# codihuston/eioku

Hardware: AMD Instinct MI355X
Metric: frames/sec (scene+detect+embed) per node (higher is better)
Workload: dtype f16

## Files before the change

eioku_amd/csrc/knn.hip:

```cpp
#include "common.h"
#include "select.h"

#include <cstdlib>

#include <cfloat>

using namespace eioku;

namespace {

constexpr int kQT = 32;
constexpr int kRT = 32;
constexpr int kWaves = 4;

template <int K>
struct TopK {
  float v[K];
  int id[K];
  __device__ __forceinline__ void init() {
#pragma unroll
    for (int p = 0; p < K; ++p) {
      v[p] = FLT_MAX;
      id[p] = 0x7FFFFFFF;
    }
// ... 262 lines not shown
  const float ra = a - __uint_as_float(ua & 0xFFFF0000u), rb = b - __uint_as_float(ub & 0xFFFF0000u);
  lo = (__float_as_uint(ra) >> 16) | (__float_as_uint(rb) & 0xFFFF0000u);
}

template <int K, int D>
__global__ __launch_bounds__(256, 1) void k_flat_l2_bf(KnnArgs a) {
  if (a.gate && *a.gate == 0) return;
  constexpr int KC = D < 128 ? D : 128;
  constexpr int NCH = D / KC;
  constexpr int NS = KC / 16;
  constexpr int PPR = KC / 8;
  constexpr int UPR = 2 * PPR;
  constexpr int TILE_U = kRT * UPR;
  constexpr int SPT = kRT * (KC / 4) / 256;
  constexpr int LISTS = 2, NQ_WG = kQT * kWaves;
  constexpr size_t STAGE_B = (size_t)2 * NCH * TILE_U * 16 + (size_t)2 * kRT * 4;
  constexpr size_t MERGE_B = (size_t)NQ_WG * LISTS * K * 8;
  static_assert(KC % 16 == 0 && D % KC == 0 && (kRT * (KC / 4)) % 256 == 0, "tile shape");
  __shared__ __attribute__((aligned(16))) unsigned char smem[STAGE_B > MERGE_B ? STAGE_B : MERGE_B];
  u32x4k* lds = reinterpret_cast<u32x4k*>(smem);
  float* lnorm = reinterpret_cast<float*>(smem + (size_t)2 * NCH * TILE_U * 16);

  const int tid = threadIdx.x, lane = tid & 63, wave = tid >> 6;
  const int col = lane & 31, half = lane >> 5;
  const int qt = blockIdx.y * kWaves + wave;
  const int qi = qt * kQT + col;
  const bool qvalid = qi < a.nq;

  u32x4k Qh[D / 16], Ql[D / 16];
  {
    const float* qp = a.q + (size_t)(qvalid ? qi : 0) * D + 8 * half;
#pragma unroll
    for (int s = 0; s < D / 16; ++s) {
      const float4 v0 = *reinterpret_cast<const float4*>(qp + 16 * s);
      const float4 v1 = *reinterpret_cast<const float4*>(qp + 16 * s + 4);
      unsigned h[4], l[4];
      split_bf16x2(v0.x, v0.y, h[0], l[0]);
      split_bf16x2(v0.z, v0.w, h[1], l[1]);
      split_bf16x2(v1.x, v1.y, h[2], l[2]);
      split_bf16x2(v1.z, v1.w, h[3], l[3]);
      Qh[s] = qvalid ? u32x4k{h[0], h[1], h[2], h[3]} : u32x4k{0, 0, 0, 0};
      Ql[s] = qvalid ? u32x4k{l[0], l[1], l[2], l[3]} : u32x4k{0, 0, 0, 0};
    }
  }
  const float qn = qvalid ? a.qnorm[qi] : 0.f;
  TopK<K> top;
  top.init();

  const long long slab0 = (long long)blockIdx.x * a.slab_stride;
  const long long slab1 = min(a.n, slab0 + a.rows_per_block);
  float4 stage[2][NCH][SPT];
  float stage_n[2] = {0.f, 0.f};
  auto issue = [&](long long row0, int slot) {
#pragma unroll
    for (int ch = 0; ch < NCH; ++ch)
#pragma unroll
      for (int it = 0; it < SPT; ++it) {
        const int id = tid + 256 * it;
        long long r = row0 + id / (KC / 4);
        if (r >= slab1) r = slab1 - 1;
        stage[slot][ch][it] = *reinterpret_cast<const float4*>(a.db + (size_t)r * D + ch * KC + (id % (KC / 4)) * 4);
      }
    long long r = row0 + (tid < kRT ? tid : 0);
    if (r >= slab1) r = slab1 - 1;
    stage_n[slot] = a.dbnorm[r];
  };
  auto commit = [&](int buf, int slot) {
#pragma unroll
    for (int ch = 0; ch < NCH; ++ch)
#pragma unroll
      for (int it = 0; it < SPT; ++it) {
        const int id = tid + 256 * it;
        const int row = id / (KC / 4), fu = id % (KC / 4);
        const int p = (fu >> 1) ^ (row & (PPR - 1) & 15), sub = fu & 1;
        unsigned h0, l0, h1, l1;
        split_bf16x2(stage[slot][ch][it].x, stage[slot][ch][it].y, h0, l0);
        split_bf16x2(stage[slot][ch][it].z, stage[slot][ch][it].w, h1, l1);
        const u32x2k hi = u32x2k{h0, h1}, lo = u32x2k{l0, l1};
        unsigned char* base = reinterpret_cast<unsigned char*>(lds + (buf * NCH + ch) * TILE_U + row * UPR);
        *reinterpret_cast<u32x2k*>(base + p * 16 + sub * 8) = hi;
        *reinterpret_cast<u32x2k*>(base + (PPR + p) * 16 + sub * 8) = lo;
      }
    if (tid < kRT) lnorm[buf * kRT + tid] = stage_n[slot];
  };
  auto multiply = [&](long long row0, int buf) {
    f32x16 acc;
#pragma unroll
    for (int r = 0; r < 16; ++r) acc[r] = 0.f;
#pragma unroll
    for (int ch = 0; ch < NCH; ++ch) {
      const u32x4k* rowp = lds + (buf * NCH + ch) * TILE_U + col * UPR;
      u32x4k xh[NS], xl[NS];
#pragma unroll
      for (int s = 0; s < NS; ++s) {
        const int p = (2 * s + half) ^ (col & (PPR - 1) & 15);
        xh[s] = rowp[p];
        xl[s] = rowp[PPR + p];
      }
#pragma unroll
      for (int s = 0; s < NS; ++s) {
        const bf16x8 h = __builtin_bit_cast(bf16x8, xh[s]), l = __builtin_bit_cast(bf16x8, xl[s]);
        const bf16x8 qh = __builtin_bit_cast(bf16x8, Qh[ch * NS + s]), ql = __builtin_bit_cast(bf16x8, Ql[ch * NS + s]);
        acc = __builtin_amdgcn_mfma_f32_32x32x16_bf16(h, qh, acc, 0, 0, 0);
        acc = __builtin_amdgcn_mfma_f32_32x32x16_bf16(l, qh, acc, 0, 0, 0);
        acc = __builtin_amdgcn_mfma_f32_32x32x16_bf16(h, ql, acc, 0, 0, 0);
      }
      __builtin_amdgcn_sched_group_barrier(0x100, 4, 0);
#pragma unroll
      for (int s = 0; s < NS; ++s) {
        __builtin_amdgcn_sched_group_barrier(0x008, 3, 0);
        __builtin_amdgcn_sched_group_barrier(0x100, 2, 0);
      }
    }
#pragma unroll
    for (int r = 0; r < 16; ++r) {
      const int lr = (r & 3) + 8 * (r >> 2) + 4 * half;
      const long long row = row0 + lr;
      if (row < slab1) {
        float dist = (qn + lnorm[buf * kRT + lr]) - 2.0f * acc[r];
        dist = dist < 0.f ? 0.f : dist;
        const int id = (int)(row - slab0);
        if (top.beats_tail(dist, id)) top.insert(dist, id);
      }
    }
  };

  long long row0 = slab0;
  if (row0 < slab1) {
    issue(row0, 0);
    issue(row0 + kRT, 1);
    commit(0, 0);
  }
  __syncthreads();
  while (row0 < slab1) {
#pragma unroll
    for (int par = 0; par < 2; ++par) {
      if (row0 >= slab1) break;
      issue(row0 + 2 * kRT, par);
      multiply(row0, par);
      commit(par ^ 1, par ^ 1);
      __syncthreads();
      row0 += kRT;
    }
  }

  __syncthreads();
  float (*s_mv)[LISTS][K] = reinterpret_cast<float (*)[LISTS][K]>(smem);
  int (*s_mi)[LISTS][K] = reinterpret_cast<int (*)[LISTS][K]>(smem + (size_t)NQ_WG * LISTS * K * 4);
  {
    const int ql = wave * kQT + col;
#pragma unroll
    for (int p = 0; p < K; ++p) {
      s_mv[ql][half][p] = top.v[p];
      s_mi[ql][half][p] = top.id[p];
    }
  }
  __syncthreads();
  if (tid < NQ_WG) {
    int head[LISTS] = {0, 0};
    const int qtile = blockIdx.y * kWaves + tid / kQT;
    const size_t out = (((size_t)qtile * gridDim.x + blockIdx.x) * kQT + (tid % kQT)) * K;
    for (int p = 0; p < K; ++p) {
      float bv = FLT_MAX;
      int bi = 0x7FFFFFFF, bl = 0;
#pragma unroll
      for (int l = 0; l < LISTS; ++l) {
        if (head[l] < K) {
          const float v = s_mv[tid][l][head[l]];
          const int i = s_mi[tid][l][head[l]];
          if (v < bv || (v == bv && i < bi)) {
            bv = v;
            bi = i;
            bl = l;
          }
        }
      }
#pragma unroll
      for (int l = 0; l < LISTS; ++l)
        if (l == bl) head[l]++;
      a.pd[out + p] = bv;
      a.pi[out + p] = bi == 0x7FFFFFFF ? -1 : bi;
    }
  }
}

__global__ __launch_bounds__(256) void k_row_norms(const float* x, long long n, int d, float* out) {
  const int lane = threadIdx.x & 63;
  long long row = (blockIdx.x * 256ll + threadIdx.x) >> 6;
  const long long nw = ((long long)gridDim.x * 256) >> 6;
  for (; row < n; row += nw) {
    float s = 0.f;
    for (int c = lane * 4; c < d; c += 256) {
      const float4 v = *reinterpret_cast<const float4*>(x + (size_t)row * d + c);
      s += v.x * v.x;
      s += v.y * v.y;
      s += v.z * v.z;
      s += v.w * v.w;
    }
#pragma unroll
    for (int off = 32; off > 0; off >>= 1) s += __shfl_xor(s, off, 64);
    if (lane == 0) out[row] = s;
  }
}

template <int K>
__global__ __launch_bounds__(64) void k_topk_merge(const float* pd, const int* pi, const long long* pi64,
                                                   int L, int nq, int kin, int qstride_lists,
                                                   const long long* list_base, long long rows_per_list,
                                                   int k, float* D, long long* I, const int* gate = nullptr) {
  if (gate && *gate == 0) return;
  const int q = blockIdx.x, lane = threadIdx.x;
  SmallTop<K> top;
  top.init();
  for (int l = lane; l < L; l += 64) {
    size_t base;
    if (qstride_lists > 0) base = ((((size_t)(q / kQT) * L + l) * kQT) + (q % kQT)) * kin;
    else base = ((size_t)l * nq + q) * kin;
    for (int p = 0; p < kin; ++p) {
      const float v = pd[base + p];
      long long id;
      if (pi64) id = pi64[base + p];
      else {
        const int li = pi[base + p];
        id = li < 0 ? -1 : (long long)li + (list_base ? list_base[l] : (long long)l * rows_per_list);
      }
      if (id < 0) break;
      if (!top.better(v, id, top.v[K - 1], top.id[K - 1])) break;
      top.insert(v, id);
    }
  }
  for (int r = 0; r < k; ++r) {
    float bv = top.id[0] < 0 ? FLT_MAX : top.v[0];
    long long bi = top.id[0] < 0 ? none<long long>() : top.id[0];
    int bl = lane;
    wave_argmin(bv, bi, bl);
    const bool found = bi != none<long long>();
    if (lane == 0) {
      D[(size_t)q * k + r] = found ? bv : FLT_MAX;
      I[(size_t)q * k + r] = found ? bi : -1;
    }
    if (found && lane == bl) {
#pragma unroll
      for (int s = 0; s < K - 1; ++s) {
        top.v[s] = top.v[s + 1];
        top.id[s] = top.id[s + 1];
      }
      top.v[K - 1] = FLT_MAX;
      top.id[K - 1] = -1;
    }
  }
}

__global__ __launch_bounds__(64) void k_topk_merge_heads(const float* __restrict__ pd, const int* __restrict__ pi, int L, int kin,
                                                         long long rows_per_list, int k, float* __restrict__ D,
                                                         long long* __restrict__ I, const int* __restrict__ gate) {
  if (gate && *gate == 0) return;
  const int q = blockIdx.x, lane = threadIdx.x;
  const bool have = lane < L;
  const size_t base = ((((size_t)(q / kQT) * L + (have ? lane : 0)) * kQT) + (q % kQT)) * kin;
  const long long idb = (long long)lane * rows_per_list;
  int h = 0;
  float cv = FLT_MAX, nv = FLT_MAX;
  int ci = -1, ni = -1;
  if (have) {
    cv = pd[base];
    ci = pi[base];
    if (kin > 1) {
      nv = pd[base + 1];
      ni = pi[base + 1];
    }
  }
  for (int r = 0; r < k; ++r) {
    float bv = ci < 0 ? FLT_MAX : cv;
    long long bi = ci < 0 ? none<long long>() : (long long)ci + idb;
    int bl = lane;
    wave_argmin(bv, bi, bl);
    const bool found = bi != none<long long>();
    if (lane == 0) {
      D[(size_t)q * k + r] = found ? bv : FLT_MAX;
      I[(size_t)q * k + r] = found ? bi : -1;
    }
    if (found && lane == bl) {
      ++h;
      cv = nv;
      ci = ni;
      if (h + 1 < kin && ni >= 0) {
        nv = pd[base + h + 1];
        ni = pi[base + h + 1];
      } else {
        ni = -1;
      }
    }
  }
}

template <int D, int SPLIT>
__global__ __launch_bounds__(256) void k_split_planes(const float* __restrict__ x, long long n, long long first_tile,
                                                      const float* __restrict__ norms, u32x4k* __restrict__ hi,
                                                      float* __restrict__ hnorm, float* __restrict__ tmax) {
  constexpr int NS = D / 16, PU = NS * 64;
  const long long tile = first_tile + blockIdx.x / SPLIT;
  const int part = blockIdx.x % SPLIT;
  for (int o = part * (PU / SPLIT) + threadIdx.x; o < (part + 1) * (PU / SPLIT); o += 256) {
    const int s = o >> 6, h = (o >> 5) & 1, r = o & 31;
    const long long row = tile * 32 + r;
    float v[8];
    if (row < n) {
      const float4 a = *reinterpret_cast<const float4*>(x + (size_t)row * D + 16 * s + 8 * h);
      const float4 b = *reinterpret_cast<const float4*>(x + (size_t)row * D + 16 * s + 8 * h + 4);
      v[0] = a.x; v[1] = a.y; v[2] = a.z; v[3] = a.w; v[4] = b.x; v[5] = b.y; v[6] = b.z; v[7] = b.w;
    } else {
#pragma unroll
      for (int j = 0; j < 8; ++j) v[j] = 0.f;
    }
    unsigned hb[8];
#pragma unroll
    for (int j = 0; j < 8; ++j) hb[j] = bf16_rne_bits(v[j]);
    hi[(size_t)tile * PU + o] = u32x4k{hb[0] | (hb[1] << 16), hb[2] | (hb[3] << 16), hb[4] | (hb[5] << 16), hb[6] | (hb[7] << 16)};
  }
  if (hnorm && part == 0 && threadIdx.x < 64) {
    const int r = threadIdx.x & 31;
    const long long row = tile * 32 + r;
    const float nn = row < n ? norms[row] : 0.f;
    if (threadIdx.x < 32) hnorm[tile * 32 + r] = row < n ? 0.5f * nn : __builtin_inff();
    float m = nn < __builtin_inff() ? sqrtf(nn) : 0.f;
#pragma unroll
    for (int off = 16; off > 0; off >>= 1) m = fmaxf(m, __shfl_xor(m, off, 64));
    if (threadIdx.x == 0) tmax[tile] = m;
  }
}

struct ScanArgs {
  const u32x4k* xh;
  const float* hnorm;
  const float* tmax;
  const float* xmax;
  const u32x4k* qh;
  const float* qnorm;
  const float* tau;
  int tau_k;
  long long n, ntiles;
  long long tstride;
  int nq, nqt;
  unsigned* wl;
  int* wl_cnt;
  int wl_cap;
};

template <int D, int NW, int RT>
__global__ __launch_bounds__(NW * 64) void k_l2_scan(ScanArgs a) {
  constexpr int NS = D / 16, PU = NS * 64;
  constexpr int NDMA = (PU / 64 + NW - 1) / NW;
  extern __shared__ __attribute__((aligned(16))) unsigned char dyn_smem[];
  constexpr int NB = 4;
  u32x4k* qbuf = reinterpret_cast<u32x4k*>(dyn_smem);
  float* s_hc = reinterpret_cast<float*>(dyn_smem + (size_t)NB * PU * 16);
  float* s_sq = s_hc + a.nqt * 32;
  float* s_hx = s_sq + a.nqt * 32;
  int* s_cnt = reinterpret_cast<int*>(s_hx + NW * RT * 32);

  const int tid = threadIdx.x, lane = tid & 63;
  const int wave = __builtin_amdgcn_readfirstlane(tid >> 6);
  const int col = lane & 31, half = lane >> 5;

  for (int q = tid; q < a.nqt * 32; q += NW * 64) {
    float hc = __builtin_inff(), sq = 0.f;
    if (q < a.nq) {
      const float t = a.tau[(size_t)q * a.tau_k + (a.tau_k - 1)];
      const float qn = a.qnorm[q];
      const float nrm = sqrtf(qn) + a.xmax[0];
      hc = 0.5f * (qn - (t + 2e-5f * (1.0f + t) + 1e-6f * nrm * nrm));
      sq = 0.0078125f * 1.002f * sqrtf(qn);
    }
    s_hc[q] = hc;
    s_sq[q] = sq;
  }
  if (tid == 0) *s_cnt = 0;
  unsigned* const my_list = a.wl + (size_t)blockIdx.x * a.wl_cap * 2;

  const long long nwt = (a.ntiles + NW * RT - 1) / (NW * RT);
  auto stage_q = [&](int qt, int buf) {
#pragma unroll
    for (int j = 0; j < NDMA; ++j) {
      int u = (j * NW + wave) * 64;
      if (u >= PU) u = PU - 64;
      __builtin_amdgcn_global_load_lds((gbl_cvoid_t*)(a.qh + (size_t)qt * PU + u + lane),
                                       (lds_void_t*)(qbuf + (size_t)buf * PU + u), 16, 0, 0);
    }
  };

  u32x4k xh[RT][NS];
  float sxm[RT], hxmin[RT];
  long long wt = blockIdx.x;
  auto tile_of = [&](long long w, int i) {
    const long long t = (w * NW + wave) * RT + i;
    return (t < a.ntiles ? t : a.ntiles - 1) * a.tstride;
  };
  auto tile_min_hx = [&](long long t, int i) {
    float m = a.hnorm[t * 32 + col];
    if (half == 0) s_hx[(wave * RT + i) * 32 + col] = m;
#pragma unroll
    for (int off = 16; off > 0; off >>= 1) m = fminf(m, __shfl_xor(m, off, 64));
    return m;
  };
  const long long my_tiles = wt < nwt ? (nwt - 1 - wt) / gridDim.x + 1 : 0;
  const int total = (int)(my_tiles * a.nqt);
  if (wt < nwt) {
#pragma unroll
    for (int i = 0; i < RT; ++i) {
      const long long t = tile_of(wt, i);
#pragma unroll
      for (int s = 0; s < NS; ++s) xh[i][s] = a.xh[(size_t)t * PU + s * 64 + lane];
      sxm[i] = a.tmax[t];
      hxmin[i] = tile_min_hx(t, i);
    }
    __builtin_amdgcn_s_waitcnt(0x0f70);
    __builtin_amdgcn_sched_barrier(0);
    stage_q(0, 0);
    if (total > 1) stage_q(1 % a.nqt, 1);
  }
  int it = 0;
  int stage_qt = 2 % a.nqt;
  for (; wt < nwt; wt += gridDim.x) {
    bool own[RT];
    long long row0[RT], tn[RT];
    const long long nwt_next = wt + gridDim.x;
    const bool more_tiles = nwt_next < nwt;
#pragma unroll
    for (int i = 0; i < RT; ++i) {
      own[i] = (wt * NW + wave) * RT + i < a.ntiles;
      row0[i] = tile_of(wt, i) * 32;
      tn[i] = more_tiles ? tile_of(nwt_next, i) : 0;
    }
    for (int qt = 0; qt < a.nqt; ++qt, ++it) {
      const bool last_qt = qt == a.nqt - 1;
      const bool meet = (it & 1) == 0;
      if (meet || qt == 0) __builtin_amdgcn_s_waitcnt(0x0f70);
      if (meet) {
        __builtin_amdgcn_s_waitcnt(0xc07f);
        asm volatile("" ::: "memory");
        __builtin_amdgcn_s_barrier();
        asm volatile("" ::: "memory");
        __builtin_amdgcn_sched_barrier(0);
#pragma unroll
        for (int e = 2; e < 4; ++e) {
          if (it + e < total) stage_q(stage_qt, (it + e) & (NB - 1));
          stage_qt = stage_qt + 1 == a.nqt ? 0 : stage_qt + 1;
        }
      }
      __builtin_amdgcn_sched_barrier(0);
      const u32x4k* qb = qbuf + (size_t)(it & (NB - 1)) * PU;
      const float hcq = s_hc[qt * 32 + col];
      const float sqq = s_sq[qt * 32 + col];
      f32x16 acc[RT];
#pragma unroll
      for (int i = 0; i < RT; ++i)
#pragma unroll
        for (int r = 0; r < 16; ++r) acc[i][r] = 0.f;
      constexpr int PF = RT == 2 ? 2 : 4;
      u32x4k bh[PF];
#pragma unroll
      for (int s = 0; s < PF; ++s) bh[s] = qb[s * 64 + lane];
#pragma unroll
      for (int s = 0; s < NS; ++s) {
        const bf16x8 ch = __builtin_bit_cast(bf16x8, bh[s % PF]);
#pragma unroll
        for (int i = 0; i < RT; ++i)
          acc[i] = __builtin_amdgcn_mfma_f32_32x32x16_bf16(__builtin_bit_cast(bf16x8, xh[i][s]), ch, acc[i], 0, 0, 0);
        if (s + PF < NS) bh[s % PF] = qb[(s + PF) * 64 + lane];
        if (last_qt && more_tiles) {
#pragma unroll
          for (int i = 0; i < RT; ++i) {
            const unsigned char* base = reinterpret_cast<const unsigned char*>(a.xh) + ((size_t)tn[i] * PU + (s & ~3) * 64) * 16;
            asm volatile("global_load_dwordx4 %0, %1, %2 offset:%3" : "+v"(xh[i][s]) : "v"(lane * 16), "s"(base), "n"((s & 3) * 1024));
          }
        }
      }
      if (!last_qt) {
        __builtin_amdgcn_sched_group_barrier(0x100, PF, 0);
#pragma unroll
        for (int s = 0; s < NS; ++s) {
          __builtin_amdgcn_sched_group_barrier(0x008, RT, 0);
          __builtin_amdgcn_sched_group_barrier(0x100, 1, 0);
        }
      }
#pragma unroll
      for (int i = 0; i < RT; ++i) {
        const f32x16& c = acc[i];
        const float thr_q = hcq - sqq * sxm[i];
        auto ib = [&](int r) { return __float_as_int(c[r]); };
        const int i01 = max(max(ib(0), ib(1)), ib(2)), i23 = max(max(ib(3), ib(4)), ib(5));
        const int i45 = max(max(ib(6), ib(7)), ib(8)), i67 = max(max(ib(9), ib(10)), ib(11));
        const int i89 = max(max(ib(12), ib(13)), ib(14));
        const int imx = max(max(max(i01, i23), i45), max(max(i67, i89), ib(15)));
        const float T = hxmin[i] + thr_q;
        if ((!(T > 0.f) || imx >= __float_as_int(T)) && own[i]) {
          const int qi = qt * 32 + col;
          int h4 = 4 * half;
          asm volatile("" : "+v"(h4));
#pragma unroll
          for (int g = 0; g < 4; ++g) {
            const float4 hx = *reinterpret_cast<const float4*>(s_hx + (wave * RT + i) * 32 + 8 * g + h4);
#pragma unroll
            for (int j = 0; j < 4; ++j) {
              const float hxr = j == 0 ? hx.x : (j == 1 ? hx.y : (j == 2 ? hx.z : hx.w));
              if (c[4 * g + j] >= hxr + thr_q) {
                const int pos = atomicAdd(s_cnt, 1);
                if (pos < a.wl_cap) {
                  my_list[2 * (size_t)pos] = (unsigned)qi;
                  my_list[2 * (size_t)pos + 1] = (unsigned)((int)row0[i] + 8 * g + j + h4);
                }
              }
            }
          }
        }
      }
      if (last_qt && more_tiles) {
#pragma unroll
        for (int i = 0; i < RT; ++i) {
          sxm[i] = a.tmax[tn[i]];
          hxmin[i] = tile_min_hx(tn[i], i);
        }
      }
    }
  }
  __syncthreads();
  if (tid == 0) a.wl_cnt[blockIdx.x] = *s_cnt;
}

template <int D>
__global__ __launch_bounds__(256) void k_scan_select(const float* __restrict__ db, const float* __restrict__ q,
                                                     const int* __restrict__ cand_i, const int* __restrict__ cnt, int cap, int k,
                                                     float* __restrict__ Dout, long long* __restrict__ Iout,
                                                     int* __restrict__ overflow) {
  extern __shared__ __attribute__((aligned(16))) unsigned char dyn_smem[];
  float* sd = reinterpret_cast<float*>(dyn_smem);
  int* si = reinterpret_cast<int*>(sd + cap);
  __shared__ float s_bv[4];
  __shared__ int s_bi[4];
  const int qi = blockIdx.x, tid = threadIdx.x, lane = tid & 63;
  int c = cnt[qi];
  if (c > cap) {
    if (tid == 0) atomicOr(overflow, 1);
    c = cap;
  }
  for (int j = tid; j < c; j += 256) si[j] = cand_i[(size_t)qi * cap + j];
  __syncthreads();
  {
    constexpr int NV = D / 128, U = 4;
    const int l32 = lane & 31, hw = tid >> 5;
    float4 qv[NV];
#pragma unroll
    for (int t = 0; t < NV; ++t) qv[t] = *reinterpret_cast<const float4*>(q + (size_t)qi * D + 128 * t + 4 * l32);
    for (int j0 = hw; j0 < c; j0 += 8 * U) {
      float4 xv[U][NV];
#pragma unroll
      for (int u = 0; u < U; ++u) {
        const int j = j0 + 8 * u;
        const int r = si[j < c ? j : j0];
#pragma unroll
        for (int t = 0; t < NV; ++t) xv[u][t] = *reinterpret_cast<const float4*>(db + (size_t)r * D + 128 * t + 4 * l32);
      }
#pragma unroll
      for (int u = 0; u < U; ++u) {
        float sum = 0.f;
#pragma unroll
        for (int t = 0; t < NV; ++t) {
          float e;
          e = qv[t].x - xv[u][t].x; sum = fmaf(e, e, sum);
          e = qv[t].y - xv[u][t].y; sum = fmaf(e, e, sum);
          e = qv[t].z - xv[u][t].z; sum = fmaf(e, e, sum);
          e = qv[t].w - xv[u][t].w; sum = fmaf(e, e, sum);
        }
#pragma unroll
        for (int off = 16; off > 0; off >>= 1) sum += __shfl_xor(sum, off, 64);
        const int j = j0 + 8 * u;
        if (l32 == 0 && j < c) sd[j] = sum;
      }
    }
  }
  __syncthreads();
  float lv = -1.f;
  int li = -1;
  for (int r = 0; r < k; ++r) {
    float bv;
    int bi;
    next_after(lv, li, tid, c, 256, sd, si, bv, bi);
    block_argmin4(bv, bi, s_bv, s_bi);
    if (tid == 0) {
      Dout[(size_t)qi * k + r] = bi == none<int>() ? FLT_MAX : bv;
      Iout[(size_t)qi * k + r] = bi == none<int>() ? -1 : (long long)bi;
    }
    advance(lv, li, bv, bi);
  }
}

__global__ __launch_bounds__(1024) void k_sel_words(const unsigned* __restrict__ sel, const unsigned* __restrict__ live,
                                                    long long n, int nwords, unsigned* __restrict__ ew,
                                                    int* __restrict__ bcount) {
  __shared__ int s_cnt;
  if (threadIdx.x == 0) s_cnt = 0;
  __syncthreads();
  const int i = blockIdx.x * 1024 + threadIdx.x;
  unsigned w = 0;
  if (i < nwords) {
    w = sel ? sel[i] : 0xFFFFFFFFu;
    if (live) w &= live[i];
    const long long rem = n - (long long)i * 32;
    if (rem < 32) w &= (1u << (int)rem) - 1u;
    ew[i] = w;
  }
  const unsigned long long b = __ballot(w != 0);
  if ((threadIdx.x & 63) == 0 && b) atomicAdd(&s_cnt, __popcll(b));
  __syncthreads();
  if (threadIdx.x == 0) bcount[blockIdx.x] = s_cnt;
}

__global__ __launch_bounds__(1024) void k_sel_list(const unsigned* __restrict__ ew, const int* __restrict__ bcount, int nwords,
                                                   int* __restrict__ list, int* __restrict__ meta, long long ppm) {
  __shared__ int s_part[16], s_wc[16];
  const int tid = threadIdx.x, lane = tid & 63, wave = tid >> 6;
  int s = 0;
  for (int b = tid; b < (int)blockIdx.x; b += 1024) s += bcount[b];
#pragma unroll
  for (int off = 32; off > 0; off >>= 1) s += __shfl_xor(s, off, 64);
  const int i = blockIdx.x * 1024 + tid;
  const bool nz = i < nwords && ew[i] != 0;
  const unsigned long long b = __ballot(nz);
  if (lane == 0) {
    s_part[wave] = s;
    s_wc[wave] = __popcll(b);
  }
  __syncthreads();
  int base = 0, before = 0, mine = 0;
#pragma unroll
  for (int w = 0; w < 16; ++w) {
    base += s_part[w];
    before += w < wave ? s_wc[w] : 0;
    mine += s_wc[w];
  }
  if (nz) list[base + before + __popcll(b & ((1ull << lane) - 1ull))] = i;
  if (blockIdx.x == gridDim.x - 1 && tid == 0) {
    const int total = base + mine;
    const bool use_list = (long long)total * 1000000ll <= ppm * (long long)nwords;
    meta[0] = total;
    meta[1] = use_list ? 1 : 0;
    meta[2] = use_list ? 0 : 1;
  }
}

__global__ __launch_bounds__(256) void k_remove_ids(const long long* __restrict__ ids, long long n_ids, long long n,
                                                    long long planes_n, unsigned* __restrict__ live, float* __restrict__ norms,
                                                    float* __restrict__ hnorm, int* __restrict__ removed) {
  const long long i = blockIdx.x * 256ll + threadIdx.x;
  if (i >= n_ids) return;
  const long long id = ids[i];
  if (id < 0 || id >= n) return;
  const unsigned bit = 1u << (int)(id & 31);
  const unsigned old = atomicAnd(live + (id >> 5), ~bit);
  if (old & bit) {
    atomicAdd(removed, 1);
    norms[id] = __builtin_inff();
    if (hnorm && id < planes_n) hnorm[id] = __builtin_inff();
  }
}

}

struct eioku_index {
  int d = 0;
  long long n = 0;
  DevBuf<float> x_own;
  float* x = nullptr;
  DevBuf<float> norms;
  bool attached = false;
  long long cap() const { return attached ? n : (long long)(x_own.cap / d); }
  DevBuf<float> qbuf, qnorm, pd, dout;
  DevBuf<int> pi;
  DevBuf<long long> iout;
  DevBuf<unsigned char> xh;
  DevBuf<float> hnorm, tmax;
  DevBuf<float> xmax;
  long long planes_n = 0;
  DevBuf<unsigned char> qh;
  DevBuf<unsigned> wl;
  DevBuf<int> wl_cnt;
  DevBuf<float> tau, tau1;
  DevBuf<long long> tau_i, tau1_i;
  DevBuf<int> cand_i;
  DevBuf<int> cnt;
  int scan_mode = 1;
  int scan_cap = 4096;
  long long scan_min_rows = 262144;
  long long scan_sample = 0;
  int scan_min_nq = 1;
  int scan_prescan = 32;
  int scan_rt = 2;
  DevBuf<unsigned> live;
  DevBuf<int> removed_dev;
  long long removed = 0;
  DevBuf<long long> idbuf;
  DevBuf<unsigned> selbuf;
  DevBuf<unsigned> ew;
  DevBuf<int> tlist;
  DevBuf<int> bcount;
  DevBuf<int> meta;
  int sel_list_ppm = 32000;
};

namespace {

int norms_for(const float* x, long long n, int d, float* out, hipStream_t stream) {
  if (n == 0) return EIOKU_OK;
  long long blocks = (n * 64 + 255) / 256;
  const long long cap = (long long)num_cus() * 16;
  if (blocks > cap) blocks = cap;
  hipLaunchKernelGGL(k_row_norms, dim3((unsigned)blocks), dim3(256), 0, stream, x, n, d, out);
  EIOKU_LAUNCH_CHECK();
  return EIOKU_OK;
}

template <int K>
int launch_search_bf(int d, const KnnArgs& a, dim3 grid, hipStream_t stream) {
  switch (d) {
    case 128: hipLaunchKernelGGL((k_flat_l2_bf<K, 128>), grid, dim3(256), 0, stream, a); break;
    case 256: hipLaunchKernelGGL((k_flat_l2_bf<K, 256>), grid, dim3(256), 0, stream, a); break;
    case 384: hipLaunchKernelGGL((k_flat_l2_bf<K, 384>), grid, dim3(256), 0, stream, a); break;
    default: return -1;
  }
  EIOKU_LAUNCH_CHECK();
  return EIOKU_OK;
}

template <int K, bool WIDE, int SEL = 0>
int launch_search_k(int d, const KnnArgs& a, dim3 grid, hipStream_t stream) {
  switch (d) {
    case 64: hipLaunchKernelGGL((k_flat_l2<K, 64, WIDE, SEL>), grid, dim3(256), 0, stream, a); break;
    case 128: hipLaunchKernelGGL((k_flat_l2<K, 128, WIDE, SEL>), grid, dim3(256), 0, stream, a); break;
    case 256: hipLaunchKernelGGL((k_flat_l2<K, 256, WIDE, SEL>), grid, dim3(256), 0, stream, a); break;
    case 384: hipLaunchKernelGGL((k_flat_l2<K, 384, WIDE, SEL>), grid, dim3(256), 0, stream, a); break;
    case 512: hipLaunchKernelGGL((k_flat_l2<K, 512, WIDE, SEL>), grid, dim3(256), 0, stream, a); break;
    default:
      set_error("dimension %d not supported (64, 128, 256, 384, 512)", d);
      return EIOKU_EINVAL;
  }
  EIOKU_LAUNCH_CHECK();
  return EIOKU_OK;
}

}

extern "C" {

int eioku_index_flat_create(int d, eioku_index** out) {
  EIOKU_REQUIRE_INIT();
  EIOKU_REQUIRE(out, "NULL out");
  EIOKU_REQUIRE(d == 64 || d == 128 || d == 256 || d == 384 || d == 512,
                "dimension %d not supported (64, 128, 256, 384, 512)", d);
  auto* ix = new eioku_index();
  ix->d = d;
  *out = ix;
  return EIOKU_OK;
}

void eioku_index_destroy(eioku_index* ix) {
  if (!ix) return;
  (void)hipDeviceSynchronize();
  delete ix;
}

long long eioku_index_ntotal(const eioku_index* ix) { return ix ? ix->n : 0; }

long long eioku_index_nlive(const eioku_index* ix) { return ix ? ix->n - ix->removed : 0; }

}

namespace {

void forget_removals(eioku_index* ix) {
  if (ix->live) {
    (void)hipDeviceSynchronize();
    ix->live.reset();
  }
  ix->removed = 0;
}

}

extern "C" {

int eioku_index_reset(eioku_index* ix) {
  EIOKU_REQUIRE(ix, "NULL index");
  forget_removals(ix);
  if (ix->attached) {
    ix->x = nullptr;
    ix->attached = false;
  }
  ix->n = 0;
  ix->planes_n = 0;
  return EIOKU_OK;
}

int eioku_index_add(eioku_index* ix, const float* x, long long n, int mem, void* stream_) {
  EIOKU_REQUIRE_INIT();
  EIOKU_REQUIRE(ix && (x || n == 0) && n >= 0, "bad argument");
  EIOKU_REQUIRE(!ix->attached, "index wraps an attached buffer; reset it before add()");
  EIOKU_REQUIRE(mem == EIOKU_MEM_HOST || mem == EIOKU_MEM_DEVICE, "bad mem flag %d", mem);
  if (n == 0) return EIOKU_OK;
  hipStream_t stream = (hipStream_t)stream_;
  const long long need = ix->n + n;
  if (need > ix->cap()) {
    long long ncap = ix->cap() ? ix->cap() : 1024;
    while (ncap < need) ncap *= 2;
    DevBuf<float> nx, nn;
    DevBuf<unsigned> nl;
    EIOKU_TRY(nx.grow((size_t)ncap * ix->d));
    EIOKU_TRY(nn.grow((size_t)ncap));
    if (ix->n) {
      EIOKU_HIP_CHECK(hipMemcpyAsync(nx, ix->x, (size_t)ix->n * ix->d * sizeof(float), hipMemcpyDeviceToDevice, stream));
      EIOKU_HIP_CHECK(hipMemcpyAsync(nn, ix->norms, (size_t)ix->n * sizeof(float), hipMemcpyDeviceToDevice, stream));
    }
    if (ix->live) {
      const size_t nlw = (size_t)((ncap + 31) / 32);
      EIOKU_TRY(nl.grow(nlw));
// ... 552 lines not shown
```

Baseline: 46840.

## Switch kNN scan to 16x16x32 bf16 MFMA with matching operand layout

Replaces the 32x32x16 bf16 MFMA in the L2 scan kernel with four 16x16x32 MFMAs per step, and changes the bf16 plane packing in k_split_planes to the operand layout the new instruction expects. Threshold filtering and candidate emission are reworked for the 2x2 block accumulator layout. Index arithmetic moves to 32-bit, and per-tile scalars are made wave-uniform with readfirstlane. The query thresholds are loaded late and the scheduling barriers are interleaved to overlap loads with MFMAs. This adds register pressure and changes how the scan schedule is interleaved.

Result: no change. 46530 (-0.7%).

```diff
diff --git a/eioku_amd/csrc/knn.hip b/eioku_amd/csrc/knn.hip
--- a/eioku_amd/csrc/knn.hip
+++ b/eioku_amd/csrc/knn.hip
@@ -588,12 +588,13 @@
   const long long tile = first_tile + blockIdx.x / SPLIT;
   const int part = blockIdx.x % SPLIT;
   for (int o = part * (PU / SPLIT) + threadIdx.x; o < (part + 1) * (PU / SPLIT); o += 256) {
-    const int s = o >> 6, h = (o >> 5) & 1, r = o & 31;
-    const long long row = tile * 32 + r;
+    const int s = o >> 7, blk = (o >> 6) & 1, l = o & 63;
+    const long long row = tile * 32 + 16 * blk + (l & 15);
+    const int dim = 32 * s + 8 * (l >> 4);
     float v[8];
     if (row < n) {
-      const float4 a = *reinterpret_cast<const float4*>(x + (size_t)row * D + 16 * s + 8 * h);
-      const float4 b = *reinterpret_cast<const float4*>(x + (size_t)row * D + 16 * s + 8 * h + 4);
+      const float4 a = *reinterpret_cast<const float4*>(x + (size_t)row * D + dim);
+      const float4 b = *reinterpret_cast<const float4*>(x + (size_t)row * D + dim + 4);
       v[0] = a.x; v[1] = a.y; v[2] = a.z; v[3] = a.w; v[4] = b.x; v[5] = b.y; v[6] = b.z; v[7] = b.w;
     } else {
 #pragma unroll
@@ -633,6 +634,15 @@
   int wl_cap;
 };
 
+typedef float f32x4 __attribute__((ext_vector_type(4)));
+
+template <int OFF, int W>
+__device__ __forceinline__ int lane_bits(int lane16) {
+  int r;
+  asm volatile("v_bfe_u32 %0, %1, %2, %3" : "=v"(r) : "v"(lane16), "n"(OFF), "n"(W));
+  return r;
+}
+
 template <int D, int NW, int RT>
 __global__ __launch_bounds__(NW * 64) void k_l2_scan(ScanArgs a) {
   constexpr int NS = D / 16, PU = NS * 64;
@@ -647,7 +657,8 @@
 
   const int tid = threadIdx.x, lane = tid & 63;
   const int wave = __builtin_amdgcn_readfirstlane(tid >> 6);
-  const int col = lane & 31, half = lane >> 5;
+  int lane16 = lane * 16;
+  asm volatile("" : "+v"(lane16));
 
   for (int q = tid; q < a.nqt * 32; q += NW * 64) {
     float hc = __builtin_inff(), sq = 0.f;
@@ -664,40 +675,41 @@
   if (tid == 0) *s_cnt = 0;
   unsigned* const my_list = a.wl + (size_t)blockIdx.x * a.wl_cap * 2;
 
-  const long long nwt = (a.ntiles + NW * RT - 1) / (NW * RT);
+  const int nwt = (int)((a.ntiles + NW * RT - 1) / (NW * RT));
   auto stage_q = [&](int qt, int buf) {
 #pragma unroll
     for (int j = 0; j < NDMA; ++j) {
       int u = (j * NW + wave) * 64;
       if (u >= PU) u = PU - 64;
-      __builtin_amdgcn_global_load_lds((gbl_cvoid_t*)(a.qh + (size_t)qt * PU + u + lane),
+      __builtin_amdgcn_global_load_lds((gbl_cvoid_t*)(reinterpret_cast<const unsigned char*>(a.qh + (size_t)qt * PU + u) + (unsigned)lane16),
                                        (lds_void_t*)(qbuf + (size_t)buf * PU + u), 16, 0, 0);
     }
   };
 
-  u32x4k xh[RT][NS];
+  u32x4k xh[RT][NS + (RT * NS <= 8 ? 1 : 0)];
   float sxm[RT], hxmin[RT];
-  long long wt = blockIdx.x;
-  auto tile_of = [&](long long w, int i) {
-    const long long t = (w * NW + wave) * RT + i;
-    return (t < a.ntiles ? t : a.ntiles - 1) * a.tstride;
+  int wt = blockIdx.x;
+  auto tile_of = [&](int w, int i) {
+    const int t = (w * NW + wave) * RT + i, nt = (int)a.ntiles;
+    return (long long)(t < nt ? t : nt - 1) * a.tstride;
   };
   auto tile_min_hx = [&](long long t, int i) {
+    const int col = lane_bits<4, 5>(lane16);
     float m = a.hnorm[t * 32 + col];
-    if (half == 0) s_hx[(wave * RT + i) * 32 + col] = m;
+    if (lane_bits<9, 1>(lane16) == 0) s_hx[(wave * RT + i) * 32 + col] = m;
 #pragma unroll
     for (int off = 16; off > 0; off >>= 1) m = fminf(m, __shfl_xor(m, off, 64));
-    return m;
+    return __builtin_bit_cast(float, __builtin_amdgcn_readfirstlane(__builtin_bit_cast(int, m)));
   };
-  const long long my_tiles = wt < nwt ? (nwt - 1 - wt) / gridDim.x + 1 : 0;
-  const int total = (int)(my_tiles * a.nqt);
+  const int my_tiles = wt < nwt ? (nwt - 1 - wt) / (int)gridDim.x + 1 : 0;
+  const int total = my_tiles * a.nqt;
   if (wt < nwt) {
 #pragma unroll
     for (int i = 0; i < RT; ++i) {
       const long long t = tile_of(wt, i);
 #pragma unroll
       for (int s = 0; s < NS; ++s) xh[i][s] = a.xh[(size_t)t * PU + s * 64 + lane];
-      sxm[i] = a.tmax[t];
+      sxm[i] = __builtin_bit_cast(float, __builtin_amdgcn_readfirstlane(__builtin_bit_cast(int, a.tmax[t])));
       hxmin[i] = tile_min_hx(t, i);
     }
     __builtin_amdgcn_s_waitcnt(0x0f70);
@@ -710,11 +722,11 @@
   for (; wt < nwt; wt += gridDim.x) {
     bool own[RT];
     long long row0[RT], tn[RT];
-    const long long nwt_next = wt + gridDim.x;
+    const int nwt_next = wt + gridDim.x;
     const bool more_tiles = nwt_next < nwt;
 #pragma unroll
     for (int i = 0; i < RT; ++i) {
-      own[i] = (wt * NW + wave) * RT + i < a.ntiles;
+      own[i] = (wt * NW + wave) * RT + i < (int)a.ntiles;
       row0[i] = tile_of(wt, i) * 32;
       tn[i] = more_tiles ? tile_of(nwt_next, i) : 0;
     }
@@ -735,66 +747,82 @@
         }
       }
       __builtin_amdgcn_sched_barrier(0);
-      const u32x4k* qb = qbuf + (size_t)(it & (NB - 1)) * PU;
-      const float hcq = s_hc[qt * 32 + col];
-      const float sqq = s_sq[qt * 32 + col];
-      f32x16 acc[RT];
+      const u32x4k* qb = reinterpret_cast<const u32x4k*>(reinterpret_cast<const unsigned char*>(qbuf + (size_t)(it & (NB - 1)) * PU) +
+                                                         lane16);
+      float hcq[2], sqq[2];
+      f32x4 acc[RT][2][2];
 #pragma unroll
       for (int i = 0; i < RT; ++i)
 #pragma unroll
-        for (int r = 0; r < 16; ++r) acc[i][r] = 0.f;
+        for (int r = 0; r < 16; ++r) acc[i][r >> 3][(r >> 2) & 1][r & 3] = 0.f;
       constexpr int PF = RT == 2 ? 2 : 4;
       u32x4k bh[PF];
 #pragma unroll
-      for (int s = 0; s < PF; ++s) bh[s] = qb[s * 64 + lane];
-#pragma unroll
-      for (int s = 0; s < NS; ++s) {
-        const bf16x8 ch = __builtin_bit_cast(bf16x8, bh[s % PF]);
+      for (int u = 0; u < PF; ++u) bh[u] = qb[u * 64];
+      __builtin_amdgcn_sched_group_barrier(0x100, PF, 0);
+#pragma unroll
+      for (int u = 0; u < NS; ++u) {
+        const bf16x8 ch = __builtin_bit_cast(bf16x8, bh[u % PF]);
+        const int s2 = u >> 1, b = u & 1;
 #pragma unroll
         for (int i = 0; i < RT; ++i)
-          acc[i] = __builtin_amdgcn_mfma_f32_32x32x16_bf16(__builtin_bit_cast(bf16x8, xh[i][s]), ch, acc[i], 0, 0, 0);
-        if (s + PF < NS) bh[s % PF] = qb[(s + PF) * 64 + lane];
-        if (last_qt && more_tiles) {
-#pragma unroll
-          for (int i = 0; i < RT; ++i) {
-            const unsigned char* base = reinterpret_cast<const unsigned char*>(a.xh) + ((size_t)tn[i] * PU + (s & ~3) * 64) * 16;
-            asm volatile("global_load_dwordx4 %0, %1, %2 offset:%3" : "+v"(xh[i][s]) : "v"(lane * 16), "s"(base), "n"((s & 3) * 1024));
+#pragma unroll
+          for (int rb = 0; rb < 2; ++rb)
+            acc[i][rb][b] = __builtin_amdgcn_mfma_f32_16x16x32_bf16(__builtin_bit_cast(bf16x8, xh[i][2 * s2 + rb]), ch,
+                                                                    acc[i][rb][b], 0, 0, 0);
+        __builtin_amdgcn_sched_group_barrier(0x008, 2 * RT, 0);
+        if (u + PF < NS) {
+          bh[u % PF] = qb[(u + PF) * 64];
+          __builtin_amdgcn_sched_group_barrier(0x100, 1, 0);
+        }
+        if (u == NS - 6) {
+          const int c16 = lane_bits<4, 4>(lane16);
+#pragma unroll
+          for (int b2 = 0; b2 < 2; ++b2) {
+            hcq[b2] = s_hc[qt * 32 + 16 * b2 + c16];
+            sqq[b2] = s_sq[qt * 32 + 16 * b2 + c16];
           }
         }
-      }
-      if (!last_qt) {
-        __builtin_amdgcn_sched_group_barrier(0x100, PF, 0);
-#pragma unroll
-        for (int s = 0; s < NS; ++s) {
-          __builtin_amdgcn_sched_group_barrier(0x008, RT, 0);
-          __builtin_amdgcn_sched_group_barrier(0x100, 1, 0);
+        if (last_qt && more_tiles && b == 1) {
+#pragma unroll
+          for (int i = 0; i < RT; ++i)
+#pragma unroll
+            for (int rb = 0; rb < 2; ++rb) {
+              const int v = 2 * s2 + rb;
+              const unsigned char* base = reinterpret_cast<const unsigned char*>(a.xh) + ((size_t)tn[i] * PU + (v & ~3) * 64) * 16;
+              asm volatile("global_load_dwordx4 %0, %1, %2 offset:%3" : "+v"(xh[i][v]) : "v"(lane16), "s"(base), "n"((v & 3) * 1024));
+            }
         }
       }
 #pragma unroll
       for (int i = 0; i < RT; ++i) {
-        const f32x16& c = acc[i];
-        const float thr_q = hcq - sqq * sxm[i];
-        auto ib = [&](int r) { return __float_as_int(c[r]); };
-        const int i01 = max(max(ib(0), ib(1)), ib(2)), i23 = max(max(ib(3), ib(4)), ib(5));
-        const int i45 = max(max(ib(6), ib(7)), ib(8)), i67 = max(max(ib(9), ib(10)), ib(11));
-        const int i89 = max(max(ib(12), ib(13)), ib(14));
-        const int imx = max(max(max(i01, i23), i45), max(max(i67, i89), ib(15)));
-        const float T = hxmin[i] + thr_q;
-        if ((!(T > 0.f) || imx >= __float_as_int(T)) && own[i]) {
-          const int qi = qt * 32 + col;
-          int h4 = 4 * half;
-          asm volatile("" : "+v"(h4));
-#pragma unroll
-          for (int g = 0; g < 4; ++g) {
-            const float4 hx = *reinterpret_cast<const float4*>(s_hx + (wave * RT + i) * 32 + 8 * g + h4);
+        float thr_q[2];
+        bool hit = false;
+#pragma unroll
+        for (int b = 0; b < 2; ++b) {
+          thr_q[b] = hcq[b] - sqq[b] * sxm[i];
+          auto ib = [&](int r) { return __float_as_int(acc[i][r >> 2][b][r & 3]); };
+          const int i01 = max(max(ib(0), ib(1)), ib(2)), i23 = max(max(ib(3), ib(4)), ib(5));
+          const int imx = max(max(max(i01, i23), ib(6)), ib(7));
+          const float T = hxmin[i] + thr_q[b];
+          hit |= !(T > 0.f) || imx >= __float_as_int(T);
+        }
+        if (hit && own[i]) {
+          const int h4 = 4 * lane_bits<8, 2>(lane16), c16 = lane_bits<4, 4>(lane16);
+#pragma unroll
+          for (int rb = 0; rb < 2; ++rb) {
+            const float4 hx = *reinterpret_cast<const float4*>(s_hx + (wave * RT + i) * 32 + 16 * rb + h4);
 #pragma unroll
             for (int j = 0; j < 4; ++j) {
               const float hxr = j == 0 ? hx.x : (j == 1 ? hx.y : (j == 2 ? hx.z : hx.w));
-              if (c[4 * g + j] >= hxr + thr_q) {
-                const int pos = atomicAdd(s_cnt, 1);
-                if (pos < a.wl_cap) {
-                  my_list[2 * (size_t)pos] = (unsigned)qi;
-                  my_list[2 * (size_t)pos + 1] = (unsigned)((int)row0[i] + 8 * g + j + h4);
+#pragma unroll
+              for (int b = 0; b < 2; ++b) {
+                if (acc[i][rb][b][j] >= hxr + thr_q[b]) {
+                  const int pos = atomicAdd(s_cnt, 1);
+                  if (pos < a.wl_cap) {
+                    my_list[2 * (size_t)pos] = (unsigned)(qt * 32 + 16 * b + c16);
+                    my_list[2 * (size_t)pos + 1] = (unsigned)((int)row0[i] + 16 * rb + j + h4);
+                  }
                 }
               }
             }
@@ -802,10 +830,13 @@
         }
       }
       if (last_qt && more_tiles) {
+        int wn = nwt_next;
+        asm volatile("" : "+s"(wn));
 #pragma unroll
         for (int i = 0; i < RT; ++i) {
-          sxm[i] = a.tmax[tn[i]];
-          hxmin[i] = tile_min_hx(tn[i], i);
+          const long long t = tile_of(wn, i);
+          sxm[i] = __builtin_bit_cast(float, __builtin_amdgcn_readfirstlane(__builtin_bit_cast(int, a.tmax[t])));
+          hxmin[i] = tile_min_hx(t, i);
         }
       }
     }
```
